# rachtibat/LRP-eXplains-Transformers

Hardware: AMD Instinct MI355X
Metric: explanations/sec (full AttnLRP backward) Llama-3-8B seq=2048 (higher is better)
Workload: dtype bf16

## Files before the change

lrp-explains-transformers_amd/csrc/gemm_pp.hip:

```cpp
#include "common.hpp"

namespace {

constexpr int PP_KT = 64;
constexpr int PP_OPND = 256 * 128;

typedef __attribute__((address_space(3))) void* pp_lds_ptr_t;

#define PP_VMWAIT(N)                                                                              \
    do {                                                                                          \
        asm volatile("" ::: "memory");                                                            \
        __builtin_amdgcn_s_waitcnt(((N) & 15) | 0x70 | 0xF00 | (((N) >> 4) << 14));               \
        asm volatile("" ::: "memory");                                                            \
    } while (0)
#define PP_DSRD(dst, addr, off) asm volatile("ds_read_b128 %0, %1 offset:%2" : "=v"(dst) : "v"(addr), "n"(off))
#define PP_DSTR(dst, addr, off) asm volatile("ds_read_b64_tr_b16 %0, %1 offset:%2" : "=v"(dst) : "v"(addr), "n"(off))


template <typename TO, bool NN, int EPI, int ACT, bool SK = false, bool LEAN = false, bool RS = false>
__global__ __launch_bounds__(512, 2) void gemm_pp_kernel(
    const bf16_t* __restrict__ A, const bf16_t* __restrict__ B, TO* __restrict__ C, const bf16_t* __restrict__ bias,
    int M, int N, int K, int64_t lda, int64_t ldb, int64_t ldc, int tiles_m, int tiles_n, int kt_per_split, int64_t slab_stride, PPEpi ep) {
    extern __shared__ __attribute__((aligned(16))) char smem[];
    constexpr bool ROPE = EPI == 5 || EPI == 6;
    const int tid = threadIdx.x, lane = tid & 63;
    const int wave = __builtin_amdgcn_readfirstlane(tid >> 6);
    const int g = wave >> 2, wc = wave & 3;
    const int nkt_all = K / PP_KT;
    const int kt0 = blockIdx.y * kt_per_split;
    const int nkt = min(kt_per_split, nkt_all - kt0);
    C += (int64_t)blockIdx.y * slab_stride;
    const int ntiles = tiles_m * tiles_n;
    int tile = blockIdx.x;
    int m0, n0;
    {
        int tm, tn;
        grouped_tile(xcd_remap(tile, ntiles), tiles_m, tiles_n, tm, tn);
        m0 = tm * 256; n0 = tn * 256;
    }
    const int prow = lane >> 3, pslot = lane & 7;
    const __amdgpu_buffer_rsrc_t rsA = __builtin_amdgcn_make_buffer_rsrc((void*)A, 0, (int)((int64_t)M * lda * 2), 0x00020000);
    const int voA = (int)(prow * lda * 2) + ((pslot ^ prow) << 4);
    int soA[2][2];
    auto set_soA = [&](int m0_) {
#pragma unroll
        for (int a = 0; a < 2; ++a)
#pragma unroll
            for (int p = 0; p < 2; ++p) soA[a][p] = (int)((int64_t)(m0_ + g * 128 + a * 64 + wc * 16 + 8 * p) * lda * 2) + kt0 * 128;
    };
    set_soA(m0);
    const int64_t brows = NN ? (int64_t)K : (int64_t)N;
    const __amdgpu_buffer_rsrc_t rsB = __builtin_amdgcn_make_buffer_rsrc((void*)B, 0, (int)(brows * ldb * 2), 0x00020000);
    int voB[2], soB[4];
    if constexpr (NN) {
#pragma unroll
        for (int pp = 0; pp < 2; ++pp) {
            const int r = 2 * pp + (lane >> 5);
            const int f = 2 * ((r & 3) + 4 * (wave & 1));
            voB[pp] = (int)((lane >> 5) * ldb * 2) + (((lane & 31) ^ f) << 4);
        }
    } else {
        voB[0] = voB[1] = (int)(prow * ldb * 2) + ((pslot ^ prow) << 4);
    }
    auto set_soB = [&](int n0_) {
#pragma unroll
        for (int p = 0; p < 4; ++p)
            soB[p] = NN ? (int)(((int64_t)(kt0 * PP_KT + 8 * wave + 2 * p) * ldb + n0_) * 2) : (int)((int64_t)(n0_ + wave * 32 + 8 * p) * ldb * 2) + kt0 * 128;
    };
    set_soB(n0);
    const int bstep = NN ? (int)(PP_KT * ldb * 2) : 128;
    char* const ldsA = smem + (g * 128 + wc * 16) * 128;
    char* const ldsB = smem + 2 * PP_OPND + (NN ? wave * 8 * 512 : wave * 32 * 128);
    auto stage_A = [&](int a, int kt, int buf) {
#pragma unroll
        for (int p = 0; p < 2; ++p)
            __builtin_amdgcn_raw_ptr_buffer_load_lds(rsA, (pp_lds_ptr_t)(ldsA + buf * PP_OPND + a * 8192 + p * 1024), 16, voA,
                                                     soA[a][p] + kt * 128, 0, 0);
    };
    auto stage_B = [&](int kt, int buf) {
#pragma unroll
        for (int p = 0; p < 4; ++p)
            __builtin_amdgcn_raw_ptr_buffer_load_lds(rsB, (pp_lds_ptr_t)(ldsB + buf * PP_OPND + p * 1024), 16, voB[p & 1],
                                                     soB[p] + kt * bstep, 0, 0);
    };

    const int hi = lane >> 4;
    const unsigned rowA = (unsigned)((g * 128 + (lane & 15)) * 128);
    unsigned cA[2];
#pragma unroll
    for (int ks = 0; ks < 2; ++ks) cA[ks] = rowA + (unsigned)(((4 * ks + hi) ^ (lane & 7)) << 4);
    unsigned cB[4];
    if constexpr (NN) {
        const int i16 = lane & 15;
        const int f = 2 * (((i16 >> 2) & 3) + 4 * (hi & 1));
#pragma unroll
        for (int j = 0; j < 4; ++j)
            cB[j] = (unsigned)(2 * PP_OPND + (8 * hi + (i16 >> 2)) * 512 + (((8 * wc + 2 * j + ((i16 & 3) >> 1)) ^ f) << 4) + 8 * (i16 & 1));
    } else {
        const unsigned rowB = (unsigned)(2 * PP_OPND + ((ROPE ? (wc >> 1) * 128 + (wc & 1) * 32 : wc * 64) + (lane & 15)) * 128);
#pragma unroll
        for (int ks = 0; ks < 2; ++ks) cB[ks] = rowB + (unsigned)(((4 * ks + hi) ^ (lane & 7)) << 4);
        cB[2] = cB[3] = 0;
    }

    int nb[2] = {4, 4};
    if constexpr (SK) {
#pragma unroll
        for (int a = 0; a < 2; ++a) {
            const int r = (M - (m0 + g * 128 + a * 64) + 15) >> 4;
            nb[a] = r < 0 ? 0 : (r > 4 ? 4 : r);
        }
    }
    f32x4 acc[2][4][4];
    bf16x8 fa[4][2];
    union BFrag { bf16x8 v; bf16x4 h[2]; } fb[4][2];

    auto issue_prologue = [&]() { stage_A(0, 0, 0); stage_B(0, 0); stage_A(1, 0, 0); stage_A(0, 1, 1); stage_B(1, 1); };
    issue_prologue();
    PP_VMWAIT(8);
    for (;;) {
    const int em0 = m0, en0 = n0;
    const int mrow = em0 + g * 128 + (lane & 15);
    const int ncol = en0 + wc * 64;
    bool full = (em0 + 256 <= M) && (en0 + 256 <= N) && ((ldc & 7) == 0) && ((reinterpret_cast<uintptr_t>(C) & 15) == 0);
    if constexpr (EPI == 1) full = full && ((ep.ldc2 & 7) == 0) && ((reinterpret_cast<uintptr_t>(ep.c2) & 15) == 0);
    if constexpr (EPI == 2) full = full && ((ep.ldgu & 7) == 0) && ((reinterpret_cast<uintptr_t>(ep.gu) & 15) == 0);
    if constexpr (EPI == 3 || EPI == 4) full = full && ((ep.ldres & 7) == 0) && ((reinterpret_cast<uintptr_t>(ep.res) & 15) == 0);
    float rsv[8];
    auto load_rs = [&]() {
#pragma unroll
        for (int b = 0; b < 8; ++b) {
            const int gm = mrow + (b >> 2) * 64 + (b & 3) * 16;
            rsv[b] = ep.rs[gm < M ? gm : M - 1];
        }
    };
    if constexpr (RS && EPI != 4) load_rs();
    const int epoff = 16 * (hi & 1) + 8 * (hi >> 1);
    u32x4 rpre[4][2];
    auto issue_res = [&](int b, u32x4 (&d)[2]) {
        const bf16_t* p = ep.res + (int64_t)(mrow + (b >> 2) * 64 + (b & 3) * 16) * ep.ldres + ncol + epoff;
        d[0] = *reinterpret_cast<const u32x4*>(p);
        d[1] = *reinterpret_cast<const u32x4*>(p + 32);
    };
    if constexpr (EPI == 3) {
        if (full) { issue_res(0, rpre[0]); issue_res(1, rpre[1]); }
    }
    const int w5 = wc & 1, hb5 = (wc >> 1) * 128;
    const bool rot5 = ROPE && en0 + hb5 < ep.rope_cols;
    f32x4 tpre[2][4];
    const int lane_tab = (lane & 15) * 128 + 32 * w5 + 4 * hi;
    auto issue_tab = [&](int b, f32x4 (&d)[4]) {
        const int pos = (em0 + g * 128 + (b >> 2) * 64 + (b & 3) * 16) % ep.seq;
        const float* pc = ep.cos + (int64_t)pos * 128;
        const float* ps = ep.sin + (int64_t)pos * 128;
        d[0] = *reinterpret_cast<const f32x4*>(pc + lane_tab);
        d[1] = *reinterpret_cast<const f32x4*>(pc + lane_tab + 16);
        d[2] = *reinterpret_cast<const f32x4*>(ps + lane_tab);
        d[3] = *reinterpret_cast<const f32x4*>(ps + lane_tab + 16);
    };
#pragma unroll
    for (int a = 0; a < 2; ++a)
#pragma unroll
        for (int i = 0; i < 4; ++i)
#pragma unroll
            for (int j = 0; j < 4; ++j) acc[a][i][j] = f32x4{0.f, 0.f, 0.f, 0.f};
    __builtin_amdgcn_s_barrier();
    if (g == 1) __builtin_amdgcn_s_barrier();

#define PP_READ_A(BUF, AH)                                                                        \
    _Pragma("unroll") for (int ks = 0; ks < 2; ++ks) {                                            \
        PP_DSRD(fa[0][ks], cA[ks], (BUF) * PP_OPND + (AH) * 8192);                                \
        PP_DSRD(fa[1][ks], cA[ks], (BUF) * PP_OPND + (AH) * 8192 + 2048);                         \
        PP_DSRD(fa[2][ks], cA[ks], (BUF) * PP_OPND + (AH) * 8192 + 4096);                         \
        PP_DSRD(fa[3][ks], cA[ks], (BUF) * PP_OPND + (AH) * 8192 + 6144);                         \
    }
#define PP_READ_B(BUF)                                                                            \
    if constexpr (NN) {                                                                           \
        _Pragma("unroll") for (int j = 0; j < 4; ++j) {                                           \
            PP_DSTR(fb[j][0].h[0], cB[j], (BUF) * PP_OPND);                                       \
            PP_DSTR(fb[j][0].h[1], cB[j], (BUF) * PP_OPND + 2048);                                \
            PP_DSTR(fb[j][1].h[0], cB[j], (BUF) * PP_OPND + 16384);                               \
            PP_DSTR(fb[j][1].h[1], cB[j], (BUF) * PP_OPND + 16384 + 2048);                        \
        }                                                                                         \
    } else {                                                                                      \
        _Pragma("unroll") for (int ks = 0; ks < 2; ++ks) {                                        \
            PP_DSRD(fb[0][ks].v, cB[ks], (BUF) * PP_OPND);                                        \
            PP_DSRD(fb[1][ks].v, cB[ks], (BUF) * PP_OPND + 2048);                                 \
            PP_DSRD(fb[2][ks].v, cB[ks], (BUF) * PP_OPND + (ROPE ? 8192 : 4096));             \
            PP_DSRD(fb[3][ks].v, cB[ks], (BUF) * PP_OPND + (ROPE ? 10240 : 6144));            \
        }                                                                                         \
    }
#define PP_WAIT_A() asm volatile("s_waitcnt lgkmcnt(0)" : "+v"(fa[0][0]), "+v"(fa[0][1]), "+v"(fa[1][0]), "+v"(fa[1][1]),   \
                                 "+v"(fa[2][0]), "+v"(fa[2][1]), "+v"(fa[3][0]), "+v"(fa[3][1]) :: "memory")
#define PP_WAIT_B() asm volatile("" : "+v"(fb[0][0].v), "+v"(fb[0][1].v), "+v"(fb[1][0].v), "+v"(fb[1][1].v),                \
                                 "+v"(fb[2][0].v), "+v"(fb[2][1].v), "+v"(fb[3][0].v), "+v"(fb[3][1].v))
#define PP_MMA(AH)                                                                                \
    _Pragma("unroll") for (int ks = 0; ks < 2; ++ks)                                              \
        _Pragma("unroll") for (int i = 0; i < 4; ++i)                                             \
            if (!SK || i < nb[AH])                                                                \
                _Pragma("unroll") for (int j = 0; j < 4; ++j)                                     \
                    acc[AH][i][j] = __builtin_amdgcn_mfma_f32_16x16x32_bf16(fb[j][ks].v, fa[i][ks], acc[AH][i][j], 0, 0, 0);
#define PP_FENCE() __builtin_amdgcn_sched_barrier(0)

#define PP_KTILE(BUF)                                                                             \
    {                                                                                             \
                                                                        \
        PP_READ_B(BUF) PP_READ_A(BUF, 0)                                                          \
        if (t + 1 < nkt) { stage_A(1, t + 1, (BUF) ^ 1); PP_VMWAIT(8); }   \
        else PP_VMWAIT(0);                                     \
        PP_WAIT_A(); PP_WAIT_B(); PP_FENCE();                                                     \
        __builtin_amdgcn_s_barrier(); PP_FENCE();                                                 \
                                                                                      \
        __builtin_amdgcn_s_setprio(1); PP_MMA(0) __builtin_amdgcn_s_setprio(0); PP_FENCE();       \
        __builtin_amdgcn_s_barrier(); PP_FENCE();                                                 \
                                                                        \
        PP_READ_A(BUF, 1)                                                                         \
        if (t + 2 < nkt) { stage_A(0, t + 2, BUF); stage_B(t + 2, BUF); PP_VMWAIT(8); }   \
        else if (t + 1 < nkt) PP_VMWAIT(2);                    \
        PP_WAIT_A(); PP_FENCE();                                                                  \
        __builtin_amdgcn_s_barrier(); PP_FENCE();                                                 \
                                                                                      \
        __builtin_amdgcn_s_setprio(1); PP_MMA(1) __builtin_amdgcn_s_setprio(0); PP_FENCE();       \
        __builtin_amdgcn_s_barrier(); PP_FENCE();                                                 \
    }

    int t = 0;
    for (; t + 1 < nkt; t += 2) {
        PP_KTILE(0)
        ++t;
        PP_KTILE(1)
        --t;
    }
    if (t < nkt) PP_KTILE(0)
    bool has_next = false;
    if constexpr (RS && EPI != 4) {
#pragma unroll
        for (int b = 0; b < 8; ++b) asm volatile("" : "+v"(rsv[b]));
    }
    if constexpr (EPI == 3) {
        asm volatile("" : "+v"(rpre[0][0]), "+v"(rpre[0][1]), "+v"(rpre[1][0]), "+v"(rpre[1][1]));
    }
    if constexpr (ROPE) {
        issue_tab(0, tpre[0]); issue_tab(1, tpre[1]);
    }
    u32x2 bpre[4];
    if constexpr (EPI == 6) {
        const bf16_t* bp = bias + en0 + hb5 + 32 * w5 + 4 * hi;
#pragma unroll
        for (int j = 0; j < 4; ++j) bpre[j] = *reinterpret_cast<const u32x2*>(bp + 16 * (j & 1) + 64 * (j >> 1));
    }
    u32x4 gpre[4][4];
    auto issue_gu = [&](int b, u32x4 (&d)[4]) {
        const bf16_t* p = ep.gu + (int64_t)(mrow + (b >> 2) * 64 + (b & 3) * 16) * ep.ldgu + 2 * (int64_t)ncol + 8 * hi;
#pragma unroll
        for (int k = 0; k < 4; ++k) d[k] = *reinterpret_cast<const u32x4*>(p + 32 * k);
    };
    if constexpr (EPI == 2) {
        if (full) issue_gu(0, gpre[0]);
    }
    if constexpr (EPI == 4) {
        load_rs();
        if (full) { issue_res(0, rpre[0]); issue_res(1, rpre[1]); }
    }
    if (tile + (int)gridDim.x < ntiles) {
        tile += gridDim.x;
        int tm, tn;
        grouped_tile(xcd_remap(tile, ntiles), tiles_m, tiles_n, tm, tn);
        m0 = tm * 256; n0 = tn * 256;
        has_next = true;
        set_soA(m0);
        set_soB(n0);
        issue_prologue();
    }
    {
    const bool vec4 = ((ldc & 3) == 0) && ((reinterpret_cast<uintptr_t>(C) & 15) == 0);
    bool done = false;
    if constexpr (EPI == 2) {
        if (full) {
            bf16_t* adst = reinterpret_cast<bf16_t*>(C) + (int64_t)mrow * ldc + 2 * (int64_t)ncol + epoff;
            auto& pre = gpre;
            auto swz = [&](const f32x4& t0, const f32x4& t1) {
                bf16x2 x0 = {(bf16_t)t0[0], (bf16_t)t0[1]}, x1 = {(bf16_t)t0[2], (bf16_t)t0[3]};
                bf16x2 y0 = {(bf16_t)t1[0], (bf16_t)t1[1]}, y1 = {(bf16_t)t1[2], (bf16_t)t1[3]};
                auto s0 = __builtin_amdgcn_permlane16_swap(__builtin_bit_cast(uint32_t, x0), __builtin_bit_cast(uint32_t, y0), false, false);
                auto s1 = __builtin_amdgcn_permlane16_swap(__builtin_bit_cast(uint32_t, x1), __builtin_bit_cast(uint32_t, y1), false, false);
                return u32x4{s0[0], s1[0], s0[1], s1[1]};
            };
            issue_gu(1, pre[1]);
#pragma unroll
            for (int b = 0; b < 8; ++b) {
                bf16_t* dst = adst + (int64_t)((b >> 2) * 64 + (b & 3) * 16) * ldc;
                f32x4 ag[4], au[4];
#pragma unroll
                for (int j = 0; j < 4; ++j) {
                    const u32x4 c = pre[b & 3][j];
                    const f32x4 gm4 = acc[b >> 2][b & 3][j];
                    ag[j] = f32x4{gm4[0] * bf16_lo(c[0]), gm4[1] * bf16_hi(c[0]), gm4[2] * bf16_lo(c[1]), gm4[3] * bf16_hi(c[1])};
                    au[j] = f32x4{gm4[0] * bf16_lo(c[2]), gm4[1] * bf16_hi(c[2]), gm4[2] * bf16_lo(c[3]), gm4[3] * bf16_hi(c[3])};
                }
                u32x4 out[4] = {swz(ag[0], ag[1]), swz(au[0], au[1]), swz(ag[2], ag[3]), swz(au[2], au[3])};
                __builtin_amdgcn_sched_barrier(0);
#pragma unroll
                for (int k = 0; k < 4; ++k) *reinterpret_cast<u32x4*>(dst + 32 * k) = out[k];
                if (b == 0) { issue_gu(2, pre[2]); issue_gu(3, pre[3]); }
                else if (b == 1) { issue_gu(4, pre[0]); issue_gu(5, pre[1]); }
                else if (b == 2) issue_gu(6, pre[2]);
                else if (b == 3) issue_gu(7, pre[3]);
                __builtin_amdgcn_sched_barrier(0);
            }
            done = true;
        }
    }
    if constexpr (EPI == 3 || EPI == 4) {
        if (full) {
            bf16_t* cdst = reinterpret_cast<bf16_t*>(C) + (int64_t)mrow * ldc + ncol + epoff;
#pragma unroll
            for (int b = 0; b < 8; ++b) {
                float sq = 0.f;
                u32x4 out[2];
#pragma unroll
                for (int jj = 0; jj < 2; ++jj) {
                    const u32x4 o = rpre[b & 3][jj];
                    auto s0 = __builtin_amdgcn_permlane16_swap(o[0], o[2], false, false);
                    auto s1 = __builtin_amdgcn_permlane16_swap(o[1], o[3], false, false);
                    const bf16x2 a0 = __builtin_bit_cast(bf16x2, (uint32_t)s0[0]), a1 = __builtin_bit_cast(bf16x2, (uint32_t)s1[0]);
                    const bf16x2 b0 = __builtin_bit_cast(bf16x2, (uint32_t)s0[1]), b1 = __builtin_bit_cast(bf16x2, (uint32_t)s1[1]);
                    const f32x4 r0 = {(float)a0[0], (float)a0[1], (float)a1[0], (float)a1[1]};
                    const f32x4 r1 = {(float)b0[0], (float)b0[1], (float)b1[0], (float)b1[1]};
                    f32x4 v0 = acc[b >> 2][b & 3][2 * jj], v1 = acc[b >> 2][b & 3][2 * jj + 1];
                    if constexpr (RS) { v0 *= rsv[b]; v1 *= rsv[b]; }
                    if constexpr (EPI == 3) {
                        if (ep.c2 != nullptr) {
                            bf16x2 p0 = {(bf16_t)v0[0], (bf16_t)v0[1]}, p1 = {(bf16_t)v0[2], (bf16_t)v0[3]};
                            bf16x2 q0 = {(bf16_t)v1[0], (bf16_t)v1[1]}, q1 = {(bf16_t)v1[2], (bf16_t)v1[3]};
                            auto w0 = __builtin_amdgcn_permlane16_swap(__builtin_bit_cast(uint32_t, p0), __builtin_bit_cast(uint32_t, q0), false, false);
                            auto w1 = __builtin_amdgcn_permlane16_swap(__builtin_bit_cast(uint32_t, p1), __builtin_bit_cast(uint32_t, q1), false, false);
                            *reinterpret_cast<u32x4*>(ep.c2 + (int64_t)(mrow + (b >> 2) * 64 + (b & 3) * 16) * ep.ldc2 + ncol + epoff + 32 * jj) =
                                u32x4{w0[0], w1[0], w0[1], w1[1]};
                        }
                    }
                    v0 += r0; v1 += r1;
                    bf16x2 x0 = {(bf16_t)v0[0], (bf16_t)v0[1]}, x1 = {(bf16_t)v0[2], (bf16_t)v0[3]};
                    bf16x2 y0 = {(bf16_t)v1[0], (bf16_t)v1[1]}, y1 = {(bf16_t)v1[2], (bf16_t)v1[3]};
                    if constexpr (EPI == 3) {
#pragma unroll
                        for (int e = 0; e < 2; ++e) {
                            const float q0 = (float)x0[e], q1 = (float)x1[e], q2 = (float)y0[e], q3 = (float)y1[e];
                            sq += q0 * q0 + q1 * q1 + q2 * q2 + q3 * q3;
                        }
                    }
                    auto t0 = __builtin_amdgcn_permlane16_swap(__builtin_bit_cast(uint32_t, x0), __builtin_bit_cast(uint32_t, y0), false, false);
                    auto t1 = __builtin_amdgcn_permlane16_swap(__builtin_bit_cast(uint32_t, x1), __builtin_bit_cast(uint32_t, y1), false, false);
                    out[jj] = u32x4{t0[0], t1[0], t0[1], t1[1]};
                }
                __builtin_amdgcn_sched_barrier(0);
                bf16_t* dst = cdst + (int64_t)((b >> 2) * 64 + (b & 3) * 16) * ldc;
                *reinterpret_cast<u32x4*>(dst) = out[0];
                *reinterpret_cast<u32x4*>(dst + 32) = out[1];
                if constexpr (EPI == 3) {
                    sq += __shfl_xor(sq, 16);
                    sq += __shfl_xor(sq, 32);
                    if (hi == 0) ep.ssq[(int64_t)(ncol >> 6) * ep.ldssq + mrow + (b >> 2) * 64 + (b & 3) * 16] = sq;
                }
                if (b == 0) { issue_res(2, rpre[2]); issue_res(3, rpre[3]); }
                else if (b == 1) { issue_res(4, rpre[0]); issue_res(5, rpre[1]); }
                else if (b == 2) issue_res(6, rpre[2]);
                else if (b == 3) issue_res(7, rpre[3]);
                __builtin_amdgcn_sched_barrier(0);
            }
            done = true;
        }
    }
    if constexpr (ROPE) {
        if (full) {
            bf16_t* cdst = reinterpret_cast<bf16_t*>(C) + (int64_t)mrow * ldc + en0 + hb5 + 32 * w5 + epoff;
#pragma unroll
            for (int b = 0; b < 8; ++b) {
                f32x4 v[4];
#pragma unroll
                for (int j = 0; j < 4; ++j) {
                    v[j] = acc[b >> 2][b & 3][j] * rsv[b];
                    if constexpr (EPI == 6)
                        v[j] += f32x4{bf16_lo(bpre[j][0]), bf16_hi(bpre[j][0]), bf16_lo(bpre[j][1]), bf16_hi(bpre[j][1])};
                }
#pragma unroll
                for (int jj = 0; jj < 2; ++jj) {
                    f32x4 cs = tpre[b & 1][jj], sn = tpre[b & 1][2 + jj];
                    if (!rot5) { cs = f32x4{1.f, 1.f, 1.f, 1.f}; sn = f32x4{0.f, 0.f, 0.f, 0.f}; }
                    const f32x4 x1 = v[jj], x2 = v[jj + 2];
                    v[jj] = x1 * cs - x2 * sn;
                    v[jj + 2] = x2 * cs + x1 * sn;
                }
                u32x4 out[2];
#pragma unroll
                for (int jj = 0; jj < 2; ++jj) {
                    bf16x2 x0 = {(bf16_t)v[2 * jj][0], (bf16_t)v[2 * jj][1]}, x1 = {(bf16_t)v[2 * jj][2], (bf16_t)v[2 * jj][3]};
                    bf16x2 y0 = {(bf16_t)v[2 * jj + 1][0], (bf16_t)v[2 * jj + 1][1]}, y1 = {(bf16_t)v[2 * jj + 1][2], (bf16_t)v[2 * jj + 1][3]};
                    auto s0 = __builtin_amdgcn_permlane16_swap(__builtin_bit_cast(uint32_t, x0), __builtin_bit_cast(uint32_t, y0), false, false);
                    auto s1 = __builtin_amdgcn_permlane16_swap(__builtin_bit_cast(uint32_t, x1), __builtin_bit_cast(uint32_t, y1), false, false);
                    out[jj] = u32x4{s0[0], s1[0], s0[1], s1[1]};
                }
                __builtin_amdgcn_sched_barrier(0);
                bf16_t* dst = cdst + (int64_t)((b >> 2) * 64 + (b & 3) * 16) * ldc;
                *reinterpret_cast<u32x4*>(dst) = out[0];
                *reinterpret_cast<u32x4*>(dst + 64) = out[1];
                if (b + 2 < 8) issue_tab(b + 2, tpre[b & 1]);
                __builtin_amdgcn_sched_barrier(0);
            }
            done = true;
        }
    }
    if (!done)
#pragma unroll
    for (int a = 0; a < 2; ++a)
#pragma unroll
        for (int i = 0; i < 4; ++i) {
            const int gm = mrow + a * 64 + i * 16;
            f32x4 v[4];
#pragma unroll
            for (int j = 0; j < 4; ++j) {
                v[j] = acc[a][i][j];
                if constexpr (RS) v[j] *= rsv[a * 4 + i];
                if constexpr (EPI == 3 || EPI == 4) {
#pragma unroll
                    for (int e = 0; e < 4; ++e) {
                        const int gn = ncol + j * 16 + 4 * hi + e;
                        if (gm < M && gn < N) {
                            if constexpr (EPI == 3) { if (ep.c2 != nullptr) ep.c2[(int64_t)gm * ep.ldc2 + gn] = (bf16_t)v[j][e]; }
                            v[j][e] += to_f32(ep.res[(int64_t)gm * ep.ldres + gn]);
                        }
                    }
                }
                if (bias) {
#pragma unroll
                    for (int e = 0; e < 4; ++e) {
                        const int gn = ncol + j * 16 + 4 * hi + e;
                        if (gn < N) v[j][e] += to_f32(bias[gn]);
                    }
                }
            }
            if constexpr (EPI == 1) {
                f32x4 mv[2], cgv[2], cuv[2];
#pragma unroll
                for (int jj = 0; jj < 2; ++jj)
#pragma unroll
                    for (int e = 0; e < 4; ++e) {
                        float m_, cg_, cu_;
                        gated_coef<LEAN, ACT>(v[jj][e], v[jj + 2][e], ep.eps_g, ep.eps_lin, m_, cg_, cu_);
                        mv[jj][e] = m_; cgv[jj][e] = cg_; cuv[jj][e] = cu_;
                    }
                const int mcol = ncol / 2;
                if (full) {
#pragma unroll
                    for (int jj = 0; jj < 2; ++jj) {
                        bf16x2 c0 = {(bf16_t)cgv[jj][0], (bf16_t)cgv[jj][1]}, c1 = {(bf16_t)cgv[jj][2], (bf16_t)cgv[jj][3]};
                        bf16x2 c2_ = {(bf16_t)cuv[jj][0], (bf16_t)cuv[jj][1]}, c3 = {(bf16_t)cuv[jj][2], (bf16_t)cuv[jj][3]};
                        u32x4 o = {__builtin_bit_cast(uint32_t, c0), __builtin_bit_cast(uint32_t, c1), __builtin_bit_cast(uint32_t, c2_),
                                   __builtin_bit_cast(uint32_t, c3)};
                        *reinterpret_cast<u32x4*>(C + (int64_t)gm * ldc + ncol + 32 * jj + 8 * hi) = o;
                    }
                    bf16x2 x0 = {(bf16_t)mv[0][0], (bf16_t)mv[0][1]}, x1 = {(bf16_t)mv[0][2], (bf16_t)mv[0][3]};
                    bf16x2 y0 = {(bf16_t)mv[1][0], (bf16_t)mv[1][1]}, y1 = {(bf16_t)mv[1][2], (bf16_t)mv[1][3]};
                    auto s0 = __builtin_amdgcn_permlane16_swap(__builtin_bit_cast(uint32_t, x0), __builtin_bit_cast(uint32_t, y0), false, false);
                    auto s1 = __builtin_amdgcn_permlane16_swap(__builtin_bit_cast(uint32_t, x1), __builtin_bit_cast(uint32_t, y1), false, false);
                    u32x4 o = {s0[0], s1[0], s0[1], s1[1]};
                    *reinterpret_cast<u32x4*>(ep.c2 + (int64_t)gm * ep.ldc2 + mcol + 16 * (hi & 1) + 8 * (hi >> 1)) = o;
                } else if (gm < M) {
#pragma unroll
                    for (int jj = 0; jj < 2; ++jj)
#pragma unroll
                        for (int e = 0; e < 4; ++e) {
                            const int ci = mcol + 16 * jj + 4 * hi + e;
                            if (2 * ci < N) {
                                ep.c2[(int64_t)gm * ep.ldc2 + ci] = (bf16_t)mv[jj][e];
                                C[(int64_t)gm * ldc + ncol + 32 * jj + 8 * hi + e] = (TO)cgv[jj][e];
                                C[(int64_t)gm * ldc + ncol + 32 * jj + 8 * hi + 4 + e] = (TO)cuv[jj][e];
                            }
                        }
                }
            }
            if constexpr (EPI == 3) {
                float sq = 0.f;
#pragma unroll
                for (int j = 0; j < 4; ++j)
#pragma unroll
                    for (int e = 0; e < 4; ++e) {
                        const float q = (float)(bf16_t)v[j][e];
                        if (ncol + j * 16 + 4 * hi + e < N) sq += q * q;
                    }
                sq += __shfl_xor(sq, 16);
                sq += __shfl_xor(sq, 32);
                if (hi == 0 && gm < M && ncol < N) ep.ssq[(int64_t)(ncol >> 6) * ep.ldssq + gm] = sq;
            }
            if constexpr (EPI == 1) {
            } else if constexpr (EPI == 2) {
#pragma unroll
                for (int j = 0; j < 4; ++j) {
                    const int64_t gcol = 2 * (int64_t)ncol + 64 * (j >> 1);
#pragma unroll
                    for (int e = 0; e < 4; ++e) {
                        const int ci = 16 * (j & 1) + 4 * hi + e;
                        if (gm < M && ncol + 16 * j + 4 * hi + e < N) {
                            const bf16_t* cp = ep.gu + (int64_t)gm * ep.ldgu + 2 * (int64_t)ncol + 32 * j + 8 * hi + e;
                            C[(int64_t)gm * ldc + gcol + ci] = (TO)(v[j][e] * (float)cp[0]);
                            C[(int64_t)gm * ldc + gcol + 32 + ci] = (TO)(v[j][e] * (float)cp[4]);
                        }
                    }
                }
            } else
            if constexpr (sizeof(TO) == 4) {
#pragma unroll
                for (int j = 0; j < 4; ++j) {
                    const int gn = ncol + j * 16 + 4 * hi;
                    TO* dst = C + (int64_t)gm * ldc + gn;
                    if (gm < M) {
                        if (vec4 && gn + 3 < N) {
                            *reinterpret_cast<f32x4*>(dst) = v[j];
                        } else {
#pragma unroll
                            for (int e = 0; e < 4; ++e)
                                if (gn + e < N) dst[e] = v[j][e];
                        }
                    }
                }
            } else if (full) {
#pragma unroll
                for (int jj = 0; jj < 2; ++jj) {
                    bf16x2 x0 = {(bf16_t)v[2 * jj][0], (bf16_t)v[2 * jj][1]}, x1 = {(bf16_t)v[2 * jj][2], (bf16_t)v[2 * jj][3]};
                    bf16x2 y0 = {(bf16_t)v[2 * jj + 1][0], (bf16_t)v[2 * jj + 1][1]}, y1 = {(bf16_t)v[2 * jj + 1][2], (bf16_t)v[2 * jj + 1][3]};
                    auto s0 = __builtin_amdgcn_permlane16_swap(__builtin_bit_cast(uint32_t, x0), __builtin_bit_cast(uint32_t, y0), false, false);
                    auto s1 = __builtin_amdgcn_permlane16_swap(__builtin_bit_cast(uint32_t, x1), __builtin_bit_cast(uint32_t, y1), false, false);
                    u32x4 o = {s0[0], s1[0], s0[1], s1[1]};
                    *reinterpret_cast<u32x4*>(C + (int64_t)gm * ldc + ncol + 32 * jj + 16 * (hi & 1) + 8 * (hi >> 1)) = o;
                }
            } else if (gm < M) {
#pragma unroll
                for (int j = 0; j < 4; ++j)
#pragma unroll
                    for (int e = 0; e < 4; ++e) {
                        const int gn = ncol + j * 16 + 4 * hi + e;
                        if (gn < N) C[(int64_t)gm * ldc + gn] = (bf16_t)v[j][e];
                    }
            }
        }
    }
    if constexpr (RS) {
#pragma unroll
        for (int b = 0; b < 8; ++b) asm volatile("" :: "v"(rsv[b]));
    }
    if constexpr (ROPE) {
#pragma unroll
        for (int k = 0; k < 4; ++k) asm volatile("" :: "v"(tpre[0][k]), "v"(tpre[1][k]));
    }
    if constexpr (EPI == 6) {
#pragma unroll
        for (int j = 0; j < 4; ++j) asm volatile("" :: "v"(bpre[j]));
    }
    if (g == 0) __builtin_amdgcn_s_barrier();
    if (!has_next) break;
    if (full && sizeof(TO) == 2) {
        if constexpr (EPI == 0 || ROPE) PP_VMWAIT(24);
        else if constexpr (EPI == 1) PP_VMWAIT(32);
        else PP_VMWAIT(8);
    } else PP_VMWAIT(0);
    }
#undef PP_KTILE
#undef PP_READ_A
#undef PP_READ_B
#undef PP_WAIT_A
#undef PP_WAIT_B
#undef PP_MMA
#undef PP_FENCE
}

template <typename TO, bool NN, int EPI, int ACT = 0, bool SK = false, bool LEAN = false, bool RS = false>
int launch_pp_t(const void* A, const void* B, void* C, const void* bias, int M, int N, int K, int64_t lda, int64_t ldb, int64_t ldc,
                int splits, int kt_per_split, int64_t slab_stride, PPEpi ep, hipStream_t st) {
    const int tiles_m = (M + 255) / 256, tiles_n = (N + 255) / 256;
    int gx = tiles_m * tiles_n;
    if (splits == 1) {
        const int ncu = lrp_num_cus();
        if (gx > ncu) gx = ncu;
    }
    dim3 grid(gx, splits), block(512);
    const size_t lds = 4 * (size_t)PP_OPND;
    auto kern = gemm_pp_kernel<TO, NN, EPI, ACT, SK, LEAN, RS>;
    LRP_SET_MAX_LDS(kern, lds);
    hipLaunchKernelGGL(kern, grid, block, lds, st, (const bf16_t*)A, (const bf16_t*)B, (TO*)C, (const bf16_t*)bias, M, N, K, lda,
                       ldb, ldc, tiles_m, tiles_n, kt_per_split, slab_stride, ep);
    return lrp_check_launch();
}

}

int lrp_launch_gemm_pp(const void* A, const void* B, void* C, const void* bias, int M, int N, int K, int64_t lda, int64_t ldb,
                       int64_t ldc, int out_dtype, int nn, int splits, int kt_per_split, int64_t slab_stride, hipStream_t st) {
    const PPEpi ep{};
    if (M <= 240) {
        if (out_dtype == LRP_F32) {
            if (nn) return launch_pp_t<float, true, 0, 0, true>(A, B, C, bias, M, N, K, lda, ldb, ldc, splits, kt_per_split, slab_stride, ep, st);
            return launch_pp_t<float, false, 0, 0, true>(A, B, C, bias, M, N, K, lda, ldb, ldc, splits, kt_per_split, slab_stride, ep, st);
        }
        if (nn) return launch_pp_t<bf16_t, true, 0, 0, true>(A, B, C, bias, M, N, K, lda, ldb, ldc, splits, kt_per_split, slab_stride, ep, st);
        return launch_pp_t<bf16_t, false, 0, 0, true>(A, B, C, bias, M, N, K, lda, ldb, ldc, splits, kt_per_split, slab_stride, ep, st);
    }
    if (out_dtype == LRP_F32) {
        if (nn) return launch_pp_t<float, true, 0>(A, B, C, bias, M, N, K, lda, ldb, ldc, splits, kt_per_split, slab_stride, ep, st);
        return launch_pp_t<float, false, 0>(A, B, C, bias, M, N, K, lda, ldb, ldc, splits, kt_per_split, slab_stride, ep, st);
    }
    if (nn) return launch_pp_t<bf16_t, true, 0>(A, B, C, bias, M, N, K, lda, ldb, ldc, splits, kt_per_split, slab_stride, ep, st);
    return launch_pp_t<bf16_t, false, 0>(A, B, C, bias, M, N, K, lda, ldb, ldc, splits, kt_per_split, slab_stride, ep, st);
}

int lrp_launch_gemm_pp_fused(const PPFused& f, hipStream_t st) {
    const bool rs = f.ep.rs != nullptr, lean = f.ep.eps_g >= 1e-30f && f.ep.eps_lin == 0.f;
#define PP_FUSED(NN, EPI, ACT, LEAN, RS) \
    launch_pp_t<bf16_t, NN, EPI, ACT, false, LEAN, RS>(f.A, f.B, f.C, f.bias, f.M, f.N, f.K, f.lda, f.ldb, f.ldc, 1, f.K / PP_KT, 0, f.ep, st)
#define PP_GATED_FWD(ACT) \
    (lean ? (rs ? PP_FUSED(false, 1, ACT, true, true) : PP_FUSED(false, 1, ACT, true, false)) \
          : (rs ? PP_FUSED(false, 1, ACT, false, true) : PP_FUSED(false, 1, ACT, false, false)))
    switch (f.epi) {
        case 0: if (rs) return f.nn ? PP_FUSED(true, 0, 0, false, true) : PP_FUSED(false, 0, 0, false, true); break;
        case 1:
            if (!f.nn && f.ep.act == LRP_ACT_SILU) return PP_GATED_FWD(LRP_ACT_SILU);
            if (!f.nn && f.ep.act == LRP_ACT_GELU_TANH) return PP_GATED_FWD(LRP_ACT_GELU_TANH);
            break;
        case 2: if (f.nn && !rs) return PP_FUSED(true, 2, 0, false, false); break;
        case 3: if (!f.nn && !rs) return PP_FUSED(false, 3, 0, false, false); break;
        case 4: if (f.nn && rs) return PP_FUSED(true, 4, 0, false, true); break;
        case 5: if (!f.nn && rs) return PP_FUSED(false, 5, 0, false, true); break;
        case 6: if (!f.nn && rs) return PP_FUSED(false, 6, 0, false, true); break;
    }
#undef PP_GATED_FWD
#undef PP_FUSED
    return LRP_ESHAPE;
}
```

Measured before the change: 22.05.

## Overlap next tile's prologue with epilogue stores via peeled seam k-iterations

Adds a 'seam' path for persistent GEMM tiles. When the next tile's prologue was issued during the previous epilogue, the first two k-tiles are peeled, and their vmcnt waits are offset so that outstanding epilogue stores do not have to drain before compute resumes. The gate/up epilogue prefetch now uses inline-asm global loads with explicit waits. Residual and gate/up prefetch issue is moved ahead of the output stores. The aim is to cut the idle time at tile boundaries, at the cost of fragile hand-counted waitcnt arithmetic that could be wrong for some epilogue variants.

```diff
diff --git a/lrp-explains-transformers_amd/csrc/gemm_pp.hip b/lrp-explains-transformers_amd/csrc/gemm_pp.hip
--- a/lrp-explains-transformers_amd/csrc/gemm_pp.hip
+++ b/lrp-explains-transformers_amd/csrc/gemm_pp.hip
@@ -13,6 +13,7 @@
         __builtin_amdgcn_s_waitcnt(((N) & 15) | 0x70 | 0xF00 | (((N) >> 4) << 14));               \
         asm volatile("" ::: "memory");                                                            \
     } while (0)
+#define PP_GLD(W, dst, ptr, off) asm volatile("global_load_" W " %0, %1, off offset:%2" : "=&v"(dst) : "v"(ptr), "n"(off) : "memory")
 #define PP_DSRD(dst, addr, off) asm volatile("ds_read_b128 %0, %1 offset:%2" : "=v"(dst) : "v"(addr), "n"(off))
 #define PP_DSTR(dst, addr, off) asm volatile("ds_read_b64_tr_b16 %0, %1 offset:%2" : "=v"(dst) : "v"(addr), "n"(off))
 
@@ -118,6 +119,13 @@
     auto issue_prologue = [&]() { stage_A(0, 0, 0); stage_B(0, 0); stage_A(1, 0, 0); stage_A(0, 1, 1); stage_B(1, 1); };
     issue_prologue();
     PP_VMWAIT(8);
+    constexpr int SEAM_S = EPI == 1 ? 24 : 16;
+    constexpr bool SEAM_LANDED = EPI == 2 || EPI == 3 || EPI == 4;
+#define PP_SEAMWAIT(N)                                                                            \
+    do {                                                                                          \
+        if constexpr (!SEAM_LANDED) PP_VMWAIT((N) + SEAM_S);                                      \
+    } while (0)
+    bool seam = false;
     for (;;) {
     const int em0 = m0, en0 = n0;
     const int mrow = em0 + g * 128 + (lane & 15);
@@ -225,6 +233,39 @@
     }
 
     int t = 0;
+    if constexpr (!SK && sizeof(TO) == 2) {
+        if (seam) {
+            PP_READ_B(0) PP_READ_A(0, 0)
+            stage_A(1, 1, 1);
+            PP_SEAMWAIT(8);
+            PP_WAIT_A(); PP_WAIT_B(); PP_FENCE();
+            __builtin_amdgcn_s_barrier(); PP_FENCE();
+            __builtin_amdgcn_s_setprio(1); PP_MMA(0) __builtin_amdgcn_s_setprio(0); PP_FENCE();
+            __builtin_amdgcn_s_barrier(); PP_FENCE();
+            PP_READ_A(0, 1)
+            if (2 < nkt) { stage_A(0, 2, 0); stage_B(2, 0); PP_SEAMWAIT(8); }
+            else PP_SEAMWAIT(2);
+            PP_WAIT_A(); PP_FENCE();
+            __builtin_amdgcn_s_barrier(); PP_FENCE();
+            __builtin_amdgcn_s_setprio(1); PP_MMA(1) __builtin_amdgcn_s_setprio(0); PP_FENCE();
+            __builtin_amdgcn_s_barrier(); PP_FENCE();
+            PP_READ_B(1) PP_READ_A(1, 0)
+            if (2 < nkt) { stage_A(1, 2, 0); PP_VMWAIT(8); }
+            else PP_VMWAIT(0);
+            PP_WAIT_A(); PP_WAIT_B(); PP_FENCE();
+            __builtin_amdgcn_s_barrier(); PP_FENCE();
+            __builtin_amdgcn_s_setprio(1); PP_MMA(0) __builtin_amdgcn_s_setprio(0); PP_FENCE();
+            __builtin_amdgcn_s_barrier(); PP_FENCE();
+            PP_READ_A(1, 1)
+            if (3 < nkt) { stage_A(0, 3, 1); stage_B(3, 1); PP_VMWAIT(8); }
+            else if (2 < nkt) PP_VMWAIT(2);
+            PP_WAIT_A(); PP_FENCE();
+            __builtin_amdgcn_s_barrier(); PP_FENCE();
+            __builtin_amdgcn_s_setprio(1); PP_MMA(1) __builtin_amdgcn_s_setprio(0); PP_FENCE();
+            __builtin_amdgcn_s_barrier(); PP_FENCE();
+            t = 2;
+        }
+    }
     for (; t + 1 < nkt; t += 2) {
         PP_KTILE(0)
         ++t;
@@ -256,7 +297,13 @@
         for (int k = 0; k < 4; ++k) d[k] = *reinterpret_cast<const u32x4*>(p + 32 * k);
     };
     if constexpr (EPI == 2) {
-        if (full) issue_gu(0, gpre[0]);
+        if (full) {
+            const bf16_t* p = ep.gu + (int64_t)mrow * ep.ldgu + 2 * (int64_t)ncol + 8 * hi;
+            PP_GLD("dwordx4", gpre[0][0], p, 0);
+            PP_GLD("dwordx4", gpre[0][1], p, 64);
+            PP_GLD("dwordx4", gpre[0][2], p, 128);
+            PP_GLD("dwordx4", gpre[0][3], p, 192);
+        }
     }
     if constexpr (EPI == 4) {
         load_rs();
@@ -270,7 +317,15 @@
         has_next = true;
         set_soA(m0);
         set_soB(n0);
+        seam = !SK && sizeof(TO) == 2 && full;
         issue_prologue();
+        if constexpr (EPI == 2) PP_VMWAIT(14);
+    } else {
+        seam = false;
+        if constexpr (EPI == 2) PP_VMWAIT(0);
+    }
+    if constexpr (EPI == 2) {
+        if (full) asm volatile("" : "+v"(gpre[0][0]), "+v"(gpre[0][1]), "+v"(gpre[0][2]), "+v"(gpre[0][3]));
     }
     {
     const bool vec4 = ((ldc & 3) == 0) && ((reinterpret_cast<uintptr_t>(C) & 15) == 0);
@@ -300,12 +355,13 @@
                 }
                 u32x4 out[4] = {swz(ag[0], ag[1]), swz(au[0], au[1]), swz(ag[2], ag[3]), swz(au[2], au[3])};
                 __builtin_amdgcn_sched_barrier(0);
-#pragma unroll
-                for (int k = 0; k < 4; ++k) *reinterpret_cast<u32x4*>(dst + 32 * k) = out[k];
                 if (b == 0) { issue_gu(2, pre[2]); issue_gu(3, pre[3]); }
                 else if (b == 1) { issue_gu(4, pre[0]); issue_gu(5, pre[1]); }
                 else if (b == 2) issue_gu(6, pre[2]);
                 else if (b == 3) issue_gu(7, pre[3]);
+                __builtin_amdgcn_sched_barrier(0);
+#pragma unroll
+                for (int k = 0; k < 4; ++k) *reinterpret_cast<u32x4*>(dst + 32 * k) = out[k];
                 __builtin_amdgcn_sched_barrier(0);
             }
             done = true;
@@ -354,6 +410,11 @@
                     out[jj] = u32x4{t0[0], t1[0], t0[1], t1[1]};
                 }
                 __builtin_amdgcn_sched_barrier(0);
+                if (b == 0) { issue_res(2, rpre[2]); issue_res(3, rpre[3]); }
+                else if (b == 1) { issue_res(4, rpre[0]); issue_res(5, rpre[1]); }
+                else if (b == 2) issue_res(6, rpre[2]);
+                else if (b == 3) issue_res(7, rpre[3]);
+                __builtin_amdgcn_sched_barrier(0);
                 bf16_t* dst = cdst + (int64_t)((b >> 2) * 64 + (b & 3) * 16) * ldc;
                 *reinterpret_cast<u32x4*>(dst) = out[0];
                 *reinterpret_cast<u32x4*>(dst + 32) = out[1];
@@ -362,10 +423,6 @@
                     sq += __shfl_xor(sq, 32);
                     if (hi == 0) ep.ssq[(int64_t)(ncol >> 6) * ep.ldssq + mrow + (b >> 2) * 64 + (b & 3) * 16] = sq;
                 }
-                if (b == 0) { issue_res(2, rpre[2]); issue_res(3, rpre[3]); }
-                else if (b == 1) { issue_res(4, rpre[0]); issue_res(5, rpre[1]); }
-                else if (b == 2) issue_res(6, rpre[2]);
-                else if (b == 3) issue_res(7, rpre[3]);
                 __builtin_amdgcn_sched_barrier(0);
             }
             done = true;
@@ -558,12 +615,11 @@
     }
     if (g == 0) __builtin_amdgcn_s_barrier();
     if (!has_next) break;
-    if (full && sizeof(TO) == 2) {
-        if constexpr (EPI == 0 || ROPE) PP_VMWAIT(24);
-        else if constexpr (EPI == 1) PP_VMWAIT(32);
-        else PP_VMWAIT(8);
+    if (seam) {
+        PP_SEAMWAIT(8);
     } else PP_VMWAIT(0);
     }
+#undef PP_SEAMWAIT
 #undef PP_KTILE
 #undef PP_READ_A
 #undef PP_READ_B
```

Result: no change. 22.06 (median of 2 runs) (+0.1%).
